# manycore-research/PlankAssembly

Measured on AMD Instinct MI355X. Metric: train samples/sec (fwd+bwd+all-reduce+Adam), d_model=512 seq=1024 [value: bf16 MFMA, f32 accumulate / master weights; train.f32 / train.x3: the same step in exact f32 / f32 with bf16x3 products = the parity paths], higher is better.
Workload: dtype bf16; 1 GPU; train_complete.yaml model d_model=512 H=8 dff=1024 6+6 post-norm layers, dropout 0.2, S=1024 (MAX_INPUT_LENGTH 1025), T=128, batch 16/GPU; global_batch=16, seq_len=1024, parallelism=dp1

## Files before the change

include/plank_hip.h:

```cpp
#ifndef PLANK_HIP_H
#define PLANK_HIP_H
#include <stdint.h>

#ifdef __cplusplus
extern "C" {
#endif

#define PA_F32 0
#define PA_BF16 1

#define PA_EINVAL (-1)
#define PA_EALIGN (-2)
#define PA_ESHAPE (-3)

int pa_version(void);

typedef struct {
    const void* A; const void* B; void* C;
    const float* bias;
    const void* R;
    const void* aux;
    void* ws;
    int32_t M, N, K;
    int32_t lda, ldb, ldc, ldr, ldaux;
    int64_t sA, sB, sC, sR, sAux;
    int32_t batch;
    int32_t a_kcontig, b_kcontig;
    int32_t in_dtype, out_dtype;
    float alpha;
    int32_t relu;
    float aux_scale;
    float drop_p; uint32_t drop_seed;
    int32_t splitk;
    int32_t splitk_defer;
    int64_t sBias;
    void* C_lp;
    int32_t ldc_lp; int32_t pad_lp_;
} pa_gemm_args;
int pa_gemm(const pa_gemm_args* a, void* stream);
int pa_set_reserved_cus(int32_t n);
int pa_get_reserved_cus(void);
int pa_gemm_effective_splitk(int32_t K, int32_t in_dtype, int32_t splitk);
int pa_split_ctx_create(void** out);
void pa_split_ctx_destroy(void* ctx);
int pa_split_ctx_enter(void* ctx);
void* pa_split_ctx_current(void);
int pa_gemm_split_config(int32_t on, void* ws, int64_t bytes);
int pa_gemm_split_active(void);
int64_t pa_gemm_split_reused(void);
int pa_gemm_split_stats(int64_t* out2, int32_t reset);
void* pa_gemm_split_reserve(const void* src, int32_t rows, int32_t cols, int32_t ld, int32_t* pat);
int64_t pa_gemm_split_made_hits(void);
int pa_gemm_split_cache_create(void* buf, int64_t bytes, void** out);
void pa_gemm_split_cache_destroy(void* cache);
// ... 31 lines not shown

typedef struct {
    const float* u; const float* gamma; const float* beta;
    void* y; int32_t ldy; float eps;
    const float* zf; int32_t ldzf; int32_t y_f32;
} pa_gemm_norm_ext;
int pa_ln_fold_weights(void* Wf, float* u, float* v, const float* W, const float* bias, const float* gamma, const float* beta,
                       int32_t N, int32_t K, void* stream);
int pa_gemm_norm_a(const pa_gemm_args* args, const pa_gemm_norm_ext* ext, void* stream);
int pa_gemm_plan(const pa_gemm_args* args, const pa_gemm_norm_ext* ext, pa_gemm_plan_info* out);
int pa_ln_fold_weights_f32(float* Wf, float* u, float* v, const float* W, const float* bias, const float* gamma, const float* beta,
                           int32_t N, int32_t K, void* stream);

#define PA_MAX_GROUP 8
int pa_gemm_group(const pa_gemm_args* args, int32_t n, void* stream);

#define PA_MAX_COLSUM 8
typedef struct {
    const void* X; float* out;
    int32_t M, N, ldx, pad_;
} pa_colsum_desc;
int pa_colsum_many(const pa_colsum_desc* descs, int32_t n_desc, int32_t dtype, void* stream);

#define PA_MAX_REDUCE 16
typedef struct {
    const float* ws; float* out;
    int32_t rows, cols, ld_out, splitk;
} pa_reduce_desc;
int pa_splitk_reduce_many(const pa_reduce_desc* descs, int32_t n_desc, void* stream);

// ... 220 lines not shown
```

plankassembly_amd/_lib.py:

```python
from __future__ import annotations

import ctypes as C
import os

import torch

HERE = os.path.dirname(os.path.abspath(__file__))
LIB_PATH = os.environ.get("PLANK_HIP_LIB") or os.path.join(HERE, "libplank_hip.so")

PA_F32, PA_BF16 = 0, 1
_ERR = {-1: "PA_EINVAL (bad argument)", -2: "PA_EALIGN (misaligned pointer / leading dimension)",
        -3: "PA_ESHAPE (unsupported shape)", -4: "PA_ESTATE (bad model/workspace state)"}


class PlankHipError(RuntimeError):
    pass


class GemmArgs(C.Structure):
    _fields_ = [("A", C.c_void_p), ("B", C.c_void_p), ("C", C.c_void_p), ("bias", C.c_void_p),
                ("R", C.c_void_p), ("aux", C.c_void_p), ("ws", C.c_void_p),
                ("M", C.c_int32), ("N", C.c_int32), ("K", C.c_int32),
                ("lda", C.c_int32), ("ldb", C.c_int32), ("ldc", C.c_int32), ("ldr", C.c_int32),
                ("ldaux", C.c_int32),
                ("sA", C.c_int64), ("sB", C.c_int64), ("sC", C.c_int64), ("sR", C.c_int64), ("sAux", C.c_int64),
                ("batch", C.c_int32), ("a_kcontig", C.c_int32), ("b_kcontig", C.c_int32),
                ("in_dtype", C.c_int32), ("out_dtype", C.c_int32), ("alpha", C.c_float), ("relu", C.c_int32),
                ("aux_scale", C.c_float), ("drop_p", C.c_float), ("drop_seed", C.c_uint32),
                ("splitk", C.c_int32), ("splitk_defer", C.c_int32), ("sBias", C.c_int64),
                ("C_lp", C.c_void_p), ("ldc_lp", C.c_int32), ("pad_lp_", C.c_int32)]


class GemmNormExt(C.Structure):
    _fields_ = [("u", C.c_void_p), ("gamma", C.c_void_p), ("beta", C.c_void_p), ("y", C.c_void_p),
                ("ldy", C.c_int32), ("eps", C.c_float),
                ("zf", C.c_void_p), ("ldzf", C.c_int32), ("y_f32", C.c_int32)]


class GemmPlanInfo(C.Structure):
    _fields_ = [("kind", C.c_int32), ("tile_h", C.c_int32), ("tile_w", C.c_int32), ("grid", C.c_int32),
                ("block", C.c_int32), ("splitk", C.c_int32), ("units", C.c_int32), ("pad_", C.c_int32)]


class GemmLnArgs(C.Structure):
    _fields_ = [("A", C.c_void_p), ("W", C.c_void_p), ("bias", C.c_void_p), ("R", C.c_void_p),
# ... 75 lines not shown
            "pa_gemm_split_config": (I, [I, P, I64]),
            "pa_gemm_split_stats": (I, [P, I]),
            "pa_gemm_split_reused": (I64, []),
            "pa_gemm_split_made_hits": (I64, []),
            "pa_gemm_split_cache_hits": (I64, []),
            "pa_gemm_split_reserve": (P, [P, I, I, I, P]),
            "pa_gemm_split_cache_create": (I, [P, I64, P]),
            "pa_gemm_split_cache_destroy": (None, [P]),
            "pa_gemm_split_cache_use": (I, [P]),
            "pa_gemm_split_cache_entries": (I, [P]),
            "pa_gemm_split_cache_refresh": (I, [P, P]),
            "pa_layernorm_fwd_img": (I, [P, P, P, P, P, P, I64, I, F, I, P, I, P]),
            "pa_layernorm_bwd_can_img": (I, [I, I]),
            "pa_layernorm_bwd_partial_img": (I, [P, P, P, P, P, P, P, I, P, I64, I, I, F, U, P, I, P]),
            "pa_gemm_group": (I, [P, I, P]),
            "pa_segment_tail": (I, [P, I, I, P, I, I, P, I, P]),
            "pa_gemm_record": (I, [I]),
            "pa_gemm_recorded": (I, [P, I]),
            "pa_gemm_recorded_kinds": (I, [P, I]),
            "pa_gemm_recorded_groups": (I, [P, I]),
            "pa_splitk_reduce_many": (I, [P, I, P]),
            "pa_colsum_many": (I, [P, I, I, P]),
            "pa_colsum_ws_floats": (I64, [I, I]),
            "pa_colsum": (I, [P, I, I, I, I, P, I, P, P]),
            "pa_embed_input_fwd": (I, [P, I, P, P, P, I, I64, I, P]),
            "pa_embed_input_bwd": (I, [P, I, P, P, P, P, I, I64, I, P]),
            "pa_embed_segment_bwd": (I, [P, I, P, P, P, P, I, I64, I, P]),
            "pa_pack_rows": (I, [P, I, I, P, P, P]),
            "pa_group_rows": (I, [P, I, P]),
            "pa_embed_output_fwd": (I, [P, I, P, P, P, P, I, I, I, I, I, P]),
# ... 51 lines not shown
            "pa_decode_sample_buffers": (I, [P, P]),
            "pa_decode_prefix_ws_bytes": (I64, [P, I, I]),
            "pa_decode_prefix_begin": (I, [P, P, P, P, P, I64, P]),
            "pa_decode_prefix_set": (I, [P, P, P, P, P]),
            "pa_decode_prefix_buffers": (I, [P, P, P]),
            "pa_dec_cross_mq": (I, [P, P, P, P, P, I, I, I, I, P]),
            "pa_dec_cross_mq32": (I, [P, P, P, P, P, I, I, I, I, P]),
            "pa_dec_cross_mq_ws": (I, [P, P, P, P, P, I, I, I, I, P, I64, P]),
            "pa_dec_cross_mq_ws_bytes": (I64, [I, I]),
            "pa_dec_cross_mq32_ws": (I, [P, P, P, P, P, I, I, I, I, P, I64, P]),
            "pa_dec_self_mq32": (I, [P, P, P, P, I, I, I, I, P]),
        }
        for name, (res, args) in sig.items():
            fn = getattr(_lib, name)
            fn.restype, fn.argtypes = res, args
    return _lib


class SampleParams(C.Structure):
    _fields_ = [("seed", C.c_uint32), ("n_per_drawing", C.c_int32), ("temperature", C.c_float), ("top_k", C.c_int32),
                ("top_p", C.c_float)]


def check(rc: int, what: str):
    if rc != 0:
        msg = _ERR.get(rc, f"hipError {rc}")
        raise PlankHipError(f"{what} failed: {msg}")


def ws_bytes(name: str, *args) -> int:
# ... 21 lines not shown
```

plankassembly_amd/csrc/gemm.hip:

```cpp
#include <stdlib.h>
#include <climits>
#include <atomic>
#include <new>
#include <mutex>
#include <vector>
#include <type_traits>
#include <utility>
#include "pa_device.h"
#include <mutex>
#include <vector>
#include "../../include/plank_hip.h"
#include "gemm_common.h"

namespace {

constexpr int BM = 128, BN = 128, NT = 256;
__device__ __attribute__((aligned(16))) const uint32_t pa_zero16[4] = {0u, 0u, 0u, 0u};
typedef short s16x4 __attribute__((ext_vector_type(4)));

#ifdef PA_GEMM_TRACE
__device__ unsigned long long pa_trace[8192];
__device__ int pa_trace_n;
#define TR_DECL __shared__ unsigned long long tr_lds[1024]; int tr_n = 0
#define TR(tag) do { if (blockIdx.x == 0 && threadIdx.x == 0 && tr_n < 1022) { tr_lds[tr_n++] = (unsigned long long)(tag); tr_lds[tr_n++] = __builtin_amdgcn_s_memtime(); } } while (0)
// ... 675 lines not shown
                TR(10);
                epilogue(c0.un, st);
                TR(11);
            }
            if (!has1) break;
            if (c1.u != c0.u) load_bias(c1.un);
            c0 = c1; c1 = c2;
            if (has2) advance(c2);
            st = (st + 1) % 3;
        }
        TR_FLUSH;
    }
}

constexpr int PA_MAX_GROUP_ = 8;
struct GemmGroup { GemmP p[PA_MAX_GROUP_]; int begin[PA_MAX_GROUP_ + 1]; int n; int xcd_chunk; };
__device__ __forceinline__ const GemmP& first_problem(const GemmP& p) { return p; }
__device__ __forceinline__ const GemmP& first_problem(const GemmGroup& g) { return g.p[0]; }
__device__ __forceinline__ int total_units_of(const GemmP& p) { return p.units; }
__device__ __forceinline__ int total_units_of(const GemmGroup& g) { return g.xcd_chunk > 0 ? 8 * g.xcd_chunk : g.begin[g.n]; }

#ifdef PA_GEMM_TRACE3
__device__ unsigned long long pa_gemm3_trace[512 * 8];
__device__ unsigned long long pa_gemm3_items[64];
__device__ int pa_gemm3_nitems;
#define PA_TR3(i) do { if (threadIdx.x == 0 && blockIdx.x < 512) pa_gemm3_trace[blockIdx.x * 8 + (i)] = __builtin_readcyclecounter(); } while (0)
#else
#define PA_TR3(i) do { } while (0)
#endif
template <bool A_KC, bool B_KC, typename PT>
__global__ __launch_bounds__(NT, 1) void gemm3_kernel(PT prm) {
// ... 8 lines not shown
    __shared__ __attribute__((aligned(256))) char smem[NSTG * STAGE + 4 * EPI];
    const int tid = threadIdx.x, lane = tid & 63;
    const int wave = __builtin_amdgcn_readfirstlane(tid >> 6);
    PA_TR3(0);
    const int wm = wave >> 1, wn = wave & 1;
    const int half = lane >> 5;
    constexpr int esz = 2;

    f32x16 acc[2][2];
#pragma unroll
    for (int i = 0; i < 2; ++i)
#pragma unroll
        for (int j = 0; j < 2; ++j)
#pragma unroll
            for (int r = 0; r < 16; ++r) acc[i][j][r] = 0.f;

    uint32_t offA[TL::NLD], offB[TL::NLD];
    bool okA[TL::NLD], okB[TL::NLD];
    const char* baseA = nullptr; const char* baseB = nullptr;
    auto setup = [&](const Unit& un) {
        baseA = reinterpret_cast<const char*>(pd.A) + (size_t)un.b * pd.sA * esz;
        baseB = reinterpret_cast<const char*>(pd.B) + (size_t)un.b * pd.sB * esz;
        const int m0 = un.tile_m * BM, n0 = un.tile_n * BN;
#pragma unroll
        for (int i = 0; i < TL::NLD; ++i) {
            const int pidx = tid + i * NT;
            if constexpr (A_KC) {
                const int row = pidx / TL::NCH, ch = ((pidx % TL::NCH) ^ (row / TL::RPB)) & (TL::NCH - 1);
                okA[i] = true;
                offA[i] = (uint32_t)min(m0 + row, pd.M - 1) * (uint32_t)(pd.lda * esz) + ch * 16;
// ... 97 lines not shown
#ifdef PA_GEMM_ABLATE
    const bool dbg_nomma = pc.dbg & 1, dbg_nord = pc.dbg & 2, dbg_nodma = pc.dbg & 4, dbg_nobar = pc.dbg & 8;
#define MMA1(ACC, X, Y) do { if (!dbg_nomma) PA_MFMA(ACC, X, Y); } while (0)
#define RD1(F, st, S, W) do { if (!dbg_nord) rd1(F, st, S, W); } while (0)
#define FRAG(F, st, S) do { if (!dbg_nord) frag(F, st, S); } while (0)
#define BAR() do { if (!dbg_nobar) __builtin_amdgcn_s_barrier(); } while (0)
#define DMA(x) do { if (!dbg_nodma) { x; } } while (0)
#else
#define MMA1(ACC, X, Y) PA_MFMA(ACC, X, Y)
#define RD1(F, st, S, W) rd1(F, st, S, W)
#define FRAG(F, st, S) frag(F, st, S)
#define BAR() __builtin_amdgcn_s_barrier()
#define DMA(x) do { x; } while (0)
#endif
    int sd = 0;
    auto step = [&](u32x4 (&fc)[4], u32x4 (&fn)[4], uint32_t stn, auto SN_, auto RD_, auto DQ_) {
        constexpr bool RD = decltype(RD_)::value;
        constexpr int DQ = decltype(DQ_)::value;
        wait_frag(fc);
        MMA1(acc[0][0], fc[2], fc[0]); if constexpr (RD) RD1(fn, stn, SN_, W0{});
        MMA1(acc[0][1], fc[2], fc[1]); if constexpr (RD) RD1(fn, stn, SN_, W1{});
        if constexpr (DQ >= 0) DMA(fetch_q(sd, std::integral_constant<int, (DQ >= 0 ? DQ : 0)>{}));
        MMA1(acc[1][0], fc[3], fc[0]); if constexpr (RD) RD1(fn, stn, SN_, W2{});
        MMA1(acc[1][1], fc[3], fc[1]); if constexpr (RD) RD1(fn, stn, SN_, W3{});
    };
    using NoQ = std::integral_constant<int, -1>;

    auto epilogue = [&](const Unit& un) {
        char* stage = smem + NSTG * STAGE + wave * EPI;
        const bool slab = pc.splitk > 1;
        const size_t cbase = slab ? (size_t)un.z * pc.M * pc.ldc : (size_t)un.b * pc.sC;
        const int mw = un.tile_m * BM + wm * 64, nw = un.tile_n * BN + wn * 64;
        const int chunk = lane & 15, rsub = lane >> 4;
        const int n = nw + chunk * 4;
        const bool out_f32 = slab || pc.out_dtype == PA_F32;
        const bool has_bias = !slab && pc.bias != nullptr, has_aux = !slab && pc.aux != nullptr;
        const bool has_res = !slab && pc.R != nullptr, has_drop = !slab && pc.drop_thr != 0;
        const bool fast = pc.vec_ok && (nw + 64 <= pc.N);
        const float alpha = slab ? 1.f : pc.alpha;
// ... 126 lines not shown
                        }
                        const size_t co = cbase + (size_t)m * pc.ldc + n + e;
                        if (out_f32) reinterpret_cast<float*>(pc.C)[co] = y;
                        else reinterpret_cast<bf16*>(pc.C)[co] = (bf16)y;
                    }
                }
            }
        }
#pragma unroll
        for (int i = 0; i < 2; ++i)
#pragma unroll
            for (int j = 0; j < 2; ++j)
#pragma unroll
                for (int r = 0; r < 16; ++r) acc[i][j][r] = 0.f;
    };

    const int ustride = gridDim.x;
    auto seek = [&](int u, Unit& un, GemmP& px, int& pi) -> int {
        while (u < total_units) {
            int local = u;
            if constexpr (GROUP) {
                int g = u;
                if (prm.xcd_chunk > 0) {
                    g = (u & 7) * prm.xcd_chunk + (u >> 3);
                    if (g >= prm.begin[prm.n]) { u += ustride; continue; }
                }
                bool moved = false;
                while (g >= prm.begin[pi + 1]) { ++pi; moved = true; }
                if (moved) px = prm.p[pi];
                local = g - prm.begin[pi];
// ... 11 lines not shown
        else cd_u = seek(u, un, pd, pd_i);
        if (cd_u < total_units) {
            setup(un);
            cd_t = un.t_begin; cd_end = un.t_end;
            k_dma = un.t_begin * TL::BK;
            stepA = A_KC ? (size_t)TL::BK * esz : (size_t)TL::BK * pd.lda * esz;
            stepB = B_KC ? (size_t)TL::BK * esz : (size_t)TL::BK * pd.ldb * esz;
            kA = baseA + (A_KC ? (size_t)k_dma * esz : (size_t)k_dma * pd.lda * esz);
            kB = baseB + (B_KC ? (size_t)k_dma * esz : (size_t)k_dma * pd.ldb * esz);
        }
    };
    Unit cun;
    auto cmp_enter = [&](int u) {
        cc_u = seek(u, cun, pc, pc_i);
        cc_t = cun.t_begin; cc_end = cun.t_end;
    };
    cmp_enter(blockIdx.x);
    if (cc_u >= total_units) return;
    dma_enter(cc_u, &cun);
    int pending = 0;
    auto issue = [&]() {
        DMA(fetch(sd));
        sd = (sd + 1) & (NSTG - 1);
        ++pending;
        if (++cd_t >= cd_end) dma_enter(cd_u + ustride);
    };
    auto wait_items = [&](int younger) {
        if (younger >= 2) asm volatile("s_waitcnt vmcnt(16)" ::: "memory");
        else if (younger == 1) asm volatile("s_waitcnt vmcnt(8)" ::: "memory");
        else asm volatile("s_waitcnt vmcnt(0)" ::: "memory");
    };
    PA_TR3(1);
#pragma unroll 1
    for (int k = 0; k < 3; ++k) if (cd_u < total_units) issue();
    wait_items(pending - 1);
    __builtin_amdgcn_s_barrier();
    PA_TR3(2);
    int sc = 0;
#ifdef PA_GEMM_TRACE3
    int tr_items = 0;
#endif
    u32x4 F0[4], F1[4];
    using S0 = std::integral_constant<int, 0>; using S1 = std::integral_constant<int, 1>;
    using S2 = std::integral_constant<int, 2>; using S3 = std::integral_constant<int, 3>;
    FRAG(F0, lds0, S0{});
    auto item = [&](auto HOT_) -> bool {
        constexpr bool HOT = decltype(HOT_)::value;
        using QA = std::integral_constant<int, HOT ? 0 : -1>; using QB = std::integral_constant<int, HOT ? 1 : -1>;
        using QC = std::integral_constant<int, HOT ? 2 : -1>; using QD = std::integral_constant<int, HOT ? 3 : -1>;
        const uint32_t st = lds0 + sc * STAGE;
#ifdef PA_GEMM_TRACE3
        if (threadIdx.x == 0 && blockIdx.x == 0 && tr_items < 63) pa_gemm3_items[tr_items++] = __builtin_readcyclecounter() | (HOT ? (1ull << 63) : 0ull);
#endif
        BAR();
        if constexpr (!HOT) { if (cd_u < total_units) issue(); }
        step(F0, F1, st, S1{}, std::true_type{}, QA{});
        step(F1, F0, st, S2{}, std::true_type{}, QB{});
        step(F0, F1, st, S3{}, std::true_type{}, QC{});
        const bool has_next = HOT || pending >= 2;
        if (has_next) {
            if constexpr (HOT) { DMA(fetch_q(sd, Q3{}); fetch_done()); sd = (sd + 1) & (NSTG - 1); ++cd_t; wait_items(2); }
            else wait_items(pending - 2);
            BAR();
        }
        step(F1, F0, lds0 + ((sc + 1) & (NSTG - 1)) * STAGE, S0{}, std::true_type{}, NoQ{});
        sc = (sc + 1) & (NSTG - 1);
        if constexpr (HOT) { ++cc_t; return true; }
        else {
            if (++cc_t >= cc_end) {
                PA_TR3(3);
#ifdef PA_GEMM_TRACE3
                if (threadIdx.x == 0 && blockIdx.x == 0) { pa_gemm3_items[tr_items] = __builtin_readcyclecounter(); pa_gemm3_nitems = tr_items; }
#endif
                epilogue(cun);
#ifdef PA_GEMM_TRACE3
                PA_TR3(5);
                asm volatile("s_waitcnt vmcnt(0)" ::: "memory");
#endif
                PA_TR3(4);
                if (has_next) cmp_enter(cc_u + ustride);
            }
            --pending;
            return has_next;
        }
    };
#pragma unroll 1
    while (true) {
        int hot = (pending == 3 && cd_u == cc_u) ? (cd_end - cd_t - 1) : 0;
#pragma unroll 1
        for (; hot > 0; --hot) item(std::true_type{});
        if (!item(std::false_type{})) break;
    }
#undef PA_RD128
#undef PA_RDTR
#undef MMA1
#undef RD1
#undef FRAG
#undef BAR
#undef DMA
#undef PA_MFMA
}

__global__ __launch_bounds__(NT, 2) void gemm3s_kernel(GemmP p) {
    using T = bf16;
    constexpr int TB = 64;
    constexpr int RB = 128, NCH = 8;
// ... 1056 lines not shown
inline GemmPlan plan_fail(int status) { GemmPlan pl = GemmPlan(); pl.status = status; return pl; }
inline void plan_kernel(GemmPlan& pl, int kind, GemmKernel kernel, const pa_gemm_args& a, int tile_h, int tile_w, int batch_times_splitk,
                        UnitOrder order, int max_blocks, int block) {
    pl.kind = kind; pl.kernel = kernel; pl.tile_h = tile_h; pl.tile_w = tile_w;
    pl.t = tiling_of(a.M, a.N, tile_h, tile_w, batch_times_splitk, order);
    pl.grid = pl.t.units < max_blocks ? pl.t.units : max_blocks;
    pl.block = block;
}

GemmPlan plan_gemm(const pa_gemm_args& a, const GemmSwitches& sw, int cus) {
    if (!a.A || !a.B || !a.C || a.M <= 0 || a.N <= 0 || a.K <= 0 || a.batch <= 0) return plan_fail(PA_EINVAL);
    if (a.in_dtype != PA_F32 && a.in_dtype != PA_BF16) return plan_fail(PA_EINVAL);
    if (a.out_dtype != PA_F32 && a.out_dtype != PA_BF16) return plan_fail(PA_EINVAL);
    if (a.drop_p < 0.f || a.drop_p >= 1.f) return plan_fail(PA_EINVAL);
    if (a.C_lp && (a.out_dtype != PA_F32 || a.ldc_lp < a.N || a.ldc_lp % 4 || (reinterpret_cast<uintptr_t>(a.C_lp) & 7))) return plan_fail(PA_EINVAL);
    GemmPlan pl = GemmPlan();
    const bool bf = a.in_dtype == PA_BF16, bk32 = bf && sw.bk == 32;
    pl.bk = bf ? (bk32 ? 32 : 64) : 16;
    const int nt = (a.K + pl.bk - 1) / pl.bk;
    const int splitk = eff_splitk(nt, a.splitk);
    if (splitk > 1 && !a.ws) return plan_fail(PA_EINVAL);
    pl.splitk = splitk;
    pl.tiles_per_slice = (nt + splitk - 1) / splitk;
    const int osz = (splitk > 1 || a.out_dtype == PA_F32) ? 4 : 2, isz = bf ? 2 : 4;
    pl.vec_ok = (splitk > 1 ? vec_ok(a.ws, a.N, (long long)a.M * a.N, osz) : vec_ok(a.C, a.ldc, a.sC, osz)) && vec_ok(a.R, a.ldr, a.sR, osz) &&
                vec_ok(a.aux, a.ldaux, a.sAux, isz) && vec_ok(a.bias, 4, a.sBias, 4);
    pl.aligned = bf ? is_aligned<bf16>(&a) : is_aligned<float>(&a);
    pl.glds = ((a.K % pl.bk) == 0 || (!a.a_kcontig && !a.b_kcontig && bf && !bk32)) && !sw.noglds;

    const Tiling base = tiling_of(a.M, a.N, BM, BN, a.batch * splitk, UNITS_XCD);
// ... 27 lines not shown
    }
    if (a.C_lp && !go_skinny) return plan_fail(PA_EINVAL);
    if (go_skinny) plan_kernel(pl, PA_GEMM_KIND_SKINNY, GK_SKINNY, a, SK_T, SK_T, 1, UNITS_PLAIN, INT_MAX, 256);
    else if (go_wide) plan_kernel(pl, PA_GEMM_KIND_WIDE, GK_WIDE, a, 128, 256, a.batch, UNITS_XCD_ALWAYS, cus, NT);
    else if (go_tall) plan_kernel(pl, PA_GEMM_KIND_WIDE, GK_TALL, a, 192, 128, a.batch, UNITS_XCD, cus, NT);
    else if (go_small) plan_kernel(pl, PA_GEMM_KIND_SMALL, GK_SMALL, a, 64, 64, a.batch, UNITS_PLAIN, 2 * cus, NT);
    else if (go_v3) plan_kernel(pl, PA_GEMM_KIND_RING, GK_RING, a, BM, BN, a.batch * splitk, UNITS_XCD, cus, NT);
    else {
        const int pair_cap = sw.grid > 0 ? (sw.grid / 256) * cus + sw.grid % 256 : INT_MAX;
        plan_kernel(pl, PA_GEMM_KIND_PAIR, GK_PAIR, a, BM, BN, a.batch * splitk, UNITS_XCD, pair_cap, NT);
    }
    return pl;
}

GemmPlan plan_norm_a(const pa_gemm_args& a, const pa_gemm_norm_ext& x, const GemmSwitches& sw, int cus) {
    if (!a.A || !a.B || !a.C || !a.bias || !x.u || a.M <= 0 || a.N <= 0 || a.K <= 0) return plan_fail(PA_EINVAL);
    if ((a.in_dtype != PA_BF16 && a.in_dtype != PA_F32) || (a.out_dtype != PA_BF16 && a.out_dtype != PA_F32) || !a.a_kcontig || !a.b_kcontig) return plan_fail(PA_EINVAL);
    auto al16 = [](const void* q) { return (reinterpret_cast<uintptr_t>(q) & 15) == 0; };
    GemmPlan pl = GemmPlan();
    pl.splitk = 1;
    const bool cbu_ok = vec_ok(a.C, a.ldc, 0, a.out_dtype == PA_F32 ? 4 : 2) && al16(a.bias) && al16(x.u);
    if (a.in_dtype == PA_F32) {
        if (a.batch != 1 || a.splitk > 1 || a.R || a.aux || a.drop_p != 0.f || a.N % 32) return plan_fail(PA_ESHAPE);
        if (!x.zf || a.K != 512 || a.M > sw.skinny_rows || a.out_dtype != PA_F32 || (x.y && (!x.y_f32 || a.N < a.K))) return plan_fail(PA_ESHAPE);
        if (x.y && (!x.gamma || !x.beta || x.ldy < a.K || x.ldy % 4 || !al16(x.y))) return plan_fail(PA_EINVAL);
        if (!is_aligned<float>(&a) || x.ldzf < a.K || x.ldzf % 4 || !al16(x.zf)) return plan_fail(PA_EALIGN);
        pl.vec_ok = cbu_ok && (!x.y || (al16(x.gamma) && al16(x.beta)));
        if (!pl.vec_ok) return plan_fail(PA_EALIGN);
        plan_kernel(pl, PA_GEMM_KIND_SKINNY, GK_SKINNY, a, SK_T, SK_T, 1, UNITS_PLAIN, INT_MAX, 256);
        return pl;
    }
// ... 577 lines not shown
        if (hb) { B3 = hb->dst; ++hits; }
        else { B3 = reinterpret_cast<bf16*>(g_split.ws + off); off += up(b_el * 2); job(a->B, B3, a->K, a->N, a->ldb, (inter ? 0 : 2) + 1 - pa); }
        b[i] = *a;
        b[i].in_dtype = PA_BF16; b[i].A = A3; b[i].B = B3; b[i].K = 3 * a->K; b[i].lda = a->M; b[i].ldb = a->N;
    }
    if (tb.n) PA_LAUNCH(split_kernel, dim3(tb.begin[tb.n]), dim3(256), 0, reinterpret_cast<hipStream_t>(stream), tb);
    g_split.on.store(0, std::memory_order_relaxed);
    const int rc = pa_gemm_group(b, n, stream);
    g_split.on.store(1, std::memory_order_relaxed);
    if (rc) return rc;
    g_cnt.taken.fetch_add(n);
    g_cnt.reused.fetch_add(hits);
    *taken = true;
    return 0;
}
extern "C" int pa_gemm_group(const pa_gemm_args* args, int32_t n, void* stream) {
    if (!args || n <= 0 || n > PA_MAX_GROUP) return PA_EINVAL;
    if (split_on() && args[0].in_dtype == PA_F32) {
        bool took = false;
        const int r3 = gemm_group_split3(args, n, stream, &took);
        if (r3) return r3;
        if (took) return 0;
        return PA_EINVAL;
    }
    static_assert(PA_MAX_GROUP == PA_MAX_GROUP_, "header / kernel table size");
    GemmGroup g; g.n = n; g.begin[0] = 0;
    int valid = 0;
    for (int i = 0; i < n; ++i) {
        const pa_gemm_args* a = &args[i];
        if (!a->A || !a->B || !a->C || a->M <= 0 || a->N <= 0 || a->K <= 0) return PA_EINVAL;
        if (a->in_dtype != PA_BF16 || a->out_dtype != PA_F32 || a->a_kcontig || a->b_kcontig || a->batch != 1) return PA_EINVAL;
        if (a->bias || a->R || a->aux || a->relu || a->drop_p > 0.f || a->alpha != 1.f) return PA_EINVAL;
        if (!is_aligned<bf16>(a)) return PA_EINVAL;
        const int nt = (a->K + 63) / 64, splitk = eff_splitk(nt, a->splitk);
        if (splitk > 1 && (!a->ws || !a->splitk_defer)) return PA_EINVAL;
        GemmP& p = g.p[i];
        p = GemmP{};
        fill_operands(p, *a);
        p.splitk = splitk; p.tiles_per_slice = (nt + splitk - 1) / splitk;
        set_tiling(p, BM, BN, splitk, UNITS_PLAIN);
        if (splitk > 1) { p.C = a->ws; p.ldc = a->N; }
        p.vec_ok = vec_ok(p.C, p.ldc, 0, 4);
        g.begin[i + 1] = g.begin[i] + p.units;
        valid += p.units;
        record_args(*a);
        record_kind(PA_GEMM_KIND_RING, g_rec_ngroups);
    }
    if (g_rec) { std::lock_guard<std::mutex> lk(g_rec_mu); if (g_rec) ++g_rec_ngroups; }
    const int cus = cus_for_gemm();
    int grid = valid < cus ? valid : cus;
    g.xcd_chunk = 0;
    if (gemm_switches().dw_xcd && valid >= 64) {
        g.xcd_chunk = (valid + 7) / 8;
        grid = (grid + 7) / 8 * 8;
        if (grid > 8 * g.xcd_chunk) grid = 8 * g.xcd_chunk;
    }
// ... 505 lines not shown
```

plankassembly_amd/csrc/runtime.hip:

```cpp
#include <stdlib.h>
#include <hip/hip_runtime.h>
#include <math.h>
#include <new>
#include <string.h>
#include <vector>
#include "../../include/plank_hip.h"

#include "model.h"

namespace {

#define RC(x) do { int rc_ = (x); if (rc_) return rc_; } while (0)

struct Ctx {
    pa_model* m; void* st;
    int dt() const { return m->cfg.dtype; }
    bool gelu() const { return m->cfg.activation == 2; }
    int ffn1(const void* A, const void* W, const float* bias, void* hidden, int rows, float drop_p, uint32_t seed) const {
        const int d = m->cfg.d_model, ff = m->cfg.d_ff;
        if (!gelu()) return linear(A, d, W, bias, hidden, ff, rows, ff, d, 1, drop_p, seed);
        RC(linear(A, d, W, bias, hidden, ff, rows, ff, d, 0));
        return pa_gelu_fwd(hidden, hidden, rows, ff, ff, dt(), drop_p, seed, st);
    }

// ... 21 lines not shown
    }
    int linear_dw(const void* dY, int lddy, const void* Xin, int ldx, float* dW, float* db, int M, int N, int K) const {
        pa_gemm_args g; memset(&g, 0, sizeof(g));
        g.A = dY; g.B = Xin; g.C = dW;
        g.M = N; g.N = K; g.K = M; g.lda = lddy; g.ldb = ldx; g.ldc = K;
        g.batch = 1; g.a_kcontig = 0; g.b_kcontig = 0;
        g.in_dtype = dt(); g.out_dtype = PA_F32;
        g.alpha = 1.f; g.aux_scale = 1.f;
        const int tiles = ((N + 127) / 128) * ((K + 127) / 128);
        const bool x3 = dt() == PA_F32 && pa_gemm_split_active();
        const int ktile = (dt() == PA_BF16 || x3) ? 64 : 16;
        const int nkt = ((x3 ? 3 * M : M) + ktile - 1) / ktile;
        static const bool plan = !(getenv("PA_DW_PLAN") && atoi(getenv("PA_DW_PLAN")) == 0);
        if (plan && m->defer_ok && tiles < 256 && m->ndwq < PA_MAX_GROUP) {
            g.splitk = 0; g.ws = nullptr;
            m->dwq[m->ndwq++] = g;
            return queue_bias(dY, lddy, db, M, N);
        }
        int sk = 1;
        if (tiles < 256) {
            static const int target_env = getenv("PA_DW_UNITS") ? atoi(getenv("PA_DW_UNITS")) : 0;
            const int target = target_env > 0 ? target_env : (m->defer_ok ? 64 : 256);
            sk = target / tiles > 0 ? target / tiles : 1;
            if (sk > 16) sk = 16;
            if (sk > nkt / 4) sk = nkt / 4 > 0 ? nkt / 4 : 1;
            while (sk > 1 && (size_t)sk * N * K > m->splitws_floats) --sk;
        }
        sk = pa_gemm_effective_splitk(M, dt(), sk);
        g.splitk = sk; g.ws = m->splitws;
        const size_t need = (size_t)sk * N * K;
        if (sk > 1 && m->ndefer < PA_MAX_REDUCE && m->slab_used + need <= m->splitws_floats && (K & 3) == 0) {
            g.ws = m->splitws + m->slab_used;
            g.splitk_defer = 1;
            pa_reduce_desc& rd = m->defer[m->ndefer++];
            rd.ws = m->splitws + m->slab_used; rd.out = dW; rd.rows = N; rd.cols = K; rd.ld_out = K; rd.splitk = sk;
            m->slab_used += (need + 3) / 4 * 4;
        }
        if (m->defer_ok && g.splitk_defer == (sk > 1 ? 1 : 0) && m->ndwq < PA_MAX_GROUP) {
            m->dwq[m->ndwq++] = g;
        } else {
            RC(pa_gemm(&g, st));
        }
        return queue_bias(dY, lddy, db, M, N);
    }
    int queue_bias(const void* dY, int lddy, float* db, int M, int N) const {
        if (db) {
            const int EB = dt() == PA_BF16 ? 8 : 4;
            const bool vec = (reinterpret_cast<uintptr_t>(dY) & 15) == 0 && lddy % EB == 0 && lddy >= (N + EB - 1) / EB * EB;
            if (m->defer_ok && vec && m->ncs < PA_MAX_COLSUM) {
                pa_colsum_desc& cd = m->cs[m->ncs++];
                cd.X = dY; cd.out = db; cd.M = M; cd.N = N; cd.ldx = lddy; cd.pad_ = 0;
            } else {
                RC(pa_colsum(dY, dt(), M, N, lddy, db, 1, m->partial, st));
            }
        }
        return 0;
    }
    int linear_ln(const void* A, int lda, const void* W, const float* bias, const void* R, void* z, void* y, const float* g,
                  const float* b, float* mean, float* rstd, int M, int K, float drop_p, uint32_t seed, float eps) const {
        static const int fuse_max = getenv("PLANK_TRAIN_FUSE_LN") ? atoi(getenv("PLANK_TRAIN_FUSE_LN")) : 0;
        const int d = m->cfg.d_model;
        if (dt() == PA_BF16 && d == 512 && M <= fuse_max && M <= pa_gemm_ln_max_rows() && K % 64 == 0) {
            pa_gemm_ln_args a; memset(&a, 0, sizeof(a));
            a.A = A; a.W = W; a.bias = bias; a.R = R; a.Z = z; a.Y = y; a.gamma = g; a.beta = b; a.mean = mean; a.rstd = rstd;
// ... 394 lines not shown
        pa_gemm_args& g = m->dwq[i];
        if (g.splitk > 0) continue;
        int s = pa_gemm_effective_splitk(g.K, g.in_dtype, sk[i]);
        const size_t need = (size_t)s * g.M * g.N;
        if (s > 1 && !(m->ndefer < PA_MAX_REDUCE && m->slab_used + need <= m->splitws_floats)) s = 1;
        g.splitk = s; g.ws = m->splitws; g.splitk_defer = 0;
        if (s > 1) {
            g.ws = m->splitws + m->slab_used;
            g.splitk_defer = 1;
            pa_reduce_desc& rd = m->defer[m->ndefer++];
            rd.ws = (const float*)g.ws; rd.out = (float*)g.C; rd.rows = g.M; rd.cols = g.N; rd.ld_out = g.ldc; rd.splitk = s;
            m->slab_used += (need + 3) / 4 * 4;
        }
    }
}
int flush_segment(pa_model* m, void* q) {
    if (m->ndwq > 0) {
        plan_group(m);
        int rc = m->ndwq > 1 ? pa_gemm_group(m->dwq, m->ndwq, q) : PA_EINVAL;
        if (rc == PA_EINVAL) { rc = 0; for (int i = 0; i < m->ndwq && !rc; ++i) rc = pa_gemm(&m->dwq[i], q); }
        m->ndwq = 0;
        RC(rc);
    }
    if (m->nlnq > 0 || m->ncs > 0 || m->ndefer > 0) {
        RC(pa_segment_tail(m->lnq, m->nlnq, m->cfg.d_model, m->cs, m->ncs, m->cfg.dtype, m->defer, m->ndefer, q));
        m->nlnq = 0; m->ncs = 0; m->ndefer = 0; m->slab_used = 0;
    }
    return 0;
}
int join_side(pa_model* m, int par, void* st) {
    if (m->ev_pending[par]) {
        HC(hipStreamWaitEvent((hipStream_t)st, (hipEvent_t)m->ev_done[par], 0));
        m->ev_pending[par] = false;
    }
// ... 233 lines not shown
```

plankassembly_amd/ops.py:

```python
from __future__ import annotations

import ctypes as C
import math

import torch

from . import _lib as L


def _f32(*shape, device):
    return torch.empty(*shape, dtype=torch.float32, device=device)


def gemm(a, b, *, a_kcontig=True, b_kcontig=True, bias=None, residual=None, aux=None, aux_scale=1.0,
         relu=False, alpha=1.0, drop_p=0.0, drop_seed=0, out_dtype=None, splitk=1, out=None, defer=False, out_lp=None):
    batched = a.dim() == 3
    A3 = a if batched else a[None]
    B3 = b if b.dim() == 3 else b[None]
    batch = A3.shape[0]
    M, K = (A3.shape[1], A3.shape[2]) if a_kcontig else (A3.shape[2], A3.shape[1])
    N = B3.shape[1] if b_kcontig else B3.shape[2]
    assert (B3.shape[2] if b_kcontig else B3.shape[1]) == K
    assert A3.stride(2) == 1 and B3.stride(2) == 1
    out_dtype = out_dtype or a.dtype
# ... 23 lines not shown
    if out_lp is not None:
        g.C_lp, g.ldc_lp = out_lp.data_ptr(), out_lp.stride(-2)
    splitk = int(L.lib().pa_gemm_effective_splitk(K, L.dt(a), splitk))
    g.splitk = splitk
    ws = None
    if splitk > 1:
        ws = _f32(splitk * batch * M * N, device=a.device)
        g.ws = ws.data_ptr()
        g.splitk_defer = int(defer)
    L.check(L.lib().pa_gemm(C.byref(g), L.stream()), "pa_gemm")
    if defer and splitk > 1:
        return out, ws, splitk
    return out


def dw_group(items):
    n = len(items)
    args = (L.GemmArgs * n)()
    outs, keep, red = [], [], []
    for i, (dy, x, sk) in enumerate(items):
        rows, M = dy.shape
        N = x.shape[1]
        sk = int(L.lib().pa_gemm_effective_splitk(rows, L.dt(dy), sk))
        out = torch.empty(M, N, dtype=torch.float32, device=dy.device)
        g = args[i]
        g.A, g.B, g.C = dy.data_ptr(), x.data_ptr(), out.data_ptr()
        g.M, g.N, g.K = M, N, rows
        g.lda, g.ldb, g.ldc = dy.stride(0), x.stride(0), out.stride(0)
        g.batch, g.a_kcontig, g.b_kcontig = 1, 0, 0
        g.in_dtype, g.out_dtype = L.dt(dy), L.dt(out)
        g.alpha, g.aux_scale, g.splitk = 1.0, 1.0, sk
        if sk > 1:
            ws = _f32(sk * M * N, device=dy.device)
            g.ws, g.splitk_defer = ws.data_ptr(), 1
            keep.append(ws)
            red.append((ws, out, sk))
        outs.append(out)
    L.check(L.lib().pa_gemm_group(C.cast(args, C.c_void_p), n, L.stream()), "pa_gemm_group")
    if red:
        splitk_reduce_many(red)
    return outs


class ColsumDesc(C.Structure):
    _fields_ = [("X", C.c_void_p), ("out", C.c_void_p), ("M", C.c_int32), ("N", C.c_int32), ("ldx", C.c_int32),
                ("pad_", C.c_int32)]


def colsum_many(items):
    n = len(items)
    descs = (ColsumDesc * n)()
    for i, (x, out) in enumerate(items):
        descs[i].X, descs[i].out = x.data_ptr(), out.data_ptr()
        descs[i].M, descs[i].N, descs[i].ldx = x.shape[0], x.shape[1], x.stride(0)
    L.check(L.lib().pa_colsum_many(C.cast(descs, C.c_void_p), n, L.dt(items[0][0]), L.stream()), "pa_colsum_many")


class ReduceDesc(C.Structure):
    _fields_ = [("ws", C.c_void_p), ("out", C.c_void_p), ("rows", C.c_int32), ("cols", C.c_int32),
                ("ld_out", C.c_int32), ("splitk", C.c_int32)]


def splitk_reduce_many(items):
    n = len(items)
    descs = (ReduceDesc * n)()
    for i, (ws, out, sk) in enumerate(items):
        descs[i].ws, descs[i].out = ws.data_ptr(), out.data_ptr()
        descs[i].rows, descs[i].cols, descs[i].ld_out, descs[i].splitk = out.shape[0], out.shape[1], out.stride(0), sk
    L.check(L.lib().pa_splitk_reduce_many(C.cast(descs, C.c_void_p), n, L.stream()), "pa_splitk_reduce_many")


def colsum(x, out=None, accumulate=False):
    M, N = x.shape
    if out is None:
        out = torch.zeros(N, dtype=torch.float32, device=x.device)
    part = _f32(int(L.lib().pa_colsum_ws_floats(M, N)), device=x.device)
    L.check(L.lib().pa_colsum(L.ptr(x), L.dt(x), M, N, x.stride(0), L.ptr(out), int(accumulate), L.ptr(part),
                              L.stream()), "pa_colsum")
    return out


def _ptr_array(tensors):
# ... 295 lines not shown
```

Baseline: 3329 samples/s.

## Fuse bias-gradient column sums into grouped dW GEMM via ones-vector MFMA

Computes the bias gradient inside the grouped weight-gradient GEMM by issuing extra MFMAs against a vector of bf16 ones while the dY fragments are already in registers. Only the tile_n==0 waves accumulate it. Split-K partials go to a workspace reduced alongside the weight partials, and the fallback path returns to a separate colsum kernel. This is meant to remove the separate colsum pass that rereads dY, at the cost of extra MFMA work, more registers in the hot loop for tile_n==0 blocks, and more launch-planning logic.

New measurement: 1060 samples/s. 68.1% lower.

```diff
diff --git a/include/plank_hip.h b/include/plank_hip.h
--- a/include/plank_hip.h
+++ b/include/plank_hip.h
@@ -36,8 +36,10 @@
     int64_t sBias;
     void* C_lp;
     int32_t ldc_lp; int32_t pad_lp_;
+    float* db; float* db_ws;
 } pa_gemm_args;
 int pa_gemm(const pa_gemm_args* a, void* stream);
+int32_t pa_gemm_args_size(void);
 int pa_set_reserved_cus(int32_t n);
 int pa_get_reserved_cus(void);
 int pa_gemm_effective_splitk(int32_t K, int32_t in_dtype, int32_t splitk);
@@ -99,6 +101,7 @@
 
 #define PA_MAX_GROUP 8
 int pa_gemm_group(const pa_gemm_args* args, int32_t n, void* stream);
+int pa_gemm_group_check(const pa_gemm_args* args, int32_t n);
 
 #define PA_MAX_COLSUM 8
 typedef struct {
diff --git a/plankassembly_amd/_lib.py b/plankassembly_amd/_lib.py
--- a/plankassembly_amd/_lib.py
+++ b/plankassembly_amd/_lib.py
@@ -28,7 +28,8 @@
                 ("in_dtype", C.c_int32), ("out_dtype", C.c_int32), ("alpha", C.c_float), ("relu", C.c_int32),
                 ("aux_scale", C.c_float), ("drop_p", C.c_float), ("drop_seed", C.c_uint32),
                 ("splitk", C.c_int32), ("splitk_defer", C.c_int32), ("sBias", C.c_int64),
-                ("C_lp", C.c_void_p), ("ldc_lp", C.c_int32), ("pad_lp_", C.c_int32)]
+                ("C_lp", C.c_void_p), ("ldc_lp", C.c_int32), ("pad_lp_", C.c_int32),
+                ("db", C.c_void_p), ("db_ws", C.c_void_p)]
 
 
 class GemmNormExt(C.Structure):
@@ -134,6 +135,8 @@
             "pa_layernorm_bwd_can_img": (I, [I, I]),
             "pa_layernorm_bwd_partial_img": (I, [P, P, P, P, P, P, P, I, P, I64, I, I, F, U, P, I, P]),
             "pa_gemm_group": (I, [P, I, P]),
+            "pa_gemm_group_check": (I, [P, I]),
+            "pa_gemm_args_size": (I, []),
             "pa_segment_tail": (I, [P, I, I, P, I, I, P, I, P]),
             "pa_gemm_record": (I, [I]),
             "pa_gemm_recorded": (I, [P, I]),
@@ -215,6 +218,9 @@
         for name, (res, args) in sig.items():
             fn = getattr(_lib, name)
             fn.restype, fn.argtypes = res, args
+        if _lib.pa_gemm_args_size() != C.sizeof(GemmArgs):
+            raise PlankHipError(f"{LIB_PATH}: pa_gemm_args is {_lib.pa_gemm_args_size()} bytes, the GemmArgs mirror "
+                                f"{C.sizeof(GemmArgs)}: the library and this package are different versions")
     return _lib
 
 
diff --git a/plankassembly_amd/csrc/gemm.hip b/plankassembly_amd/csrc/gemm.hip
--- a/plankassembly_amd/csrc/gemm.hip
+++ b/plankassembly_amd/csrc/gemm.hip
@@ -713,7 +713,7 @@
 }
 
 constexpr int PA_MAX_GROUP_ = 8;
-struct GemmGroup { GemmP p[PA_MAX_GROUP_]; int begin[PA_MAX_GROUP_ + 1]; int n; int xcd_chunk; };
+struct GemmGroup { GemmP p[PA_MAX_GROUP_]; int begin[PA_MAX_GROUP_ + 1]; int n; int xcd_chunk; float* db[PA_MAX_GROUP_]; float* db_ws[PA_MAX_GROUP_]; };
 __device__ __forceinline__ const GemmP& first_problem(const GemmP& p) { return p; }
 __device__ __forceinline__ const GemmP& first_problem(const GemmGroup& g) { return g.p[0]; }
 __device__ __forceinline__ int total_units_of(const GemmP& p) { return p.units; }
@@ -752,6 +752,18 @@
         for (int j = 0; j < 2; ++j)
 #pragma unroll
             for (int r = 0; r < 16; ++r) acc[i][j][r] = 0.f;
+    f32x16 accb[2];
+    u32x4 ones;
+    bool bias_on = false;
+    float* db_c = nullptr; float* dbws_c = nullptr;
+    if constexpr (GROUP) {
+#pragma unroll
+        for (int i = 0; i < 2; ++i)
+#pragma unroll
+            for (int r = 0; r < 16; ++r) accb[i][r] = 0.f;
+#pragma unroll
+        for (int e = 0; e < 4; ++e) ones[e] = 0x3f803f80u;
+    }
 
     uint32_t offA[TL::NLD], offB[TL::NLD];
     bool okA[TL::NLD], okB[TL::NLD];
@@ -879,8 +891,9 @@
 #define DMA(x) do { x; } while (0)
 #endif
     int sd = 0;
-    auto step = [&](u32x4 (&fc)[4], u32x4 (&fn)[4], uint32_t stn, auto SN_, auto RD_, auto DQ_) {
+    auto step = [&](u32x4 (&fc)[4], u32x4 (&fn)[4], uint32_t stn, auto SN_, auto RD_, auto DQ_, auto BIAS_) {
         constexpr bool RD = decltype(RD_)::value;
+        constexpr bool BIAS = decltype(BIAS_)::value;
         constexpr int DQ = decltype(DQ_)::value;
         wait_frag(fc);
         MMA1(acc[0][0], fc[2], fc[0]); if constexpr (RD) RD1(fn, stn, SN_, W0{});
@@ -888,6 +901,7 @@
         if constexpr (DQ >= 0) DMA(fetch_q(sd, std::integral_constant<int, (DQ >= 0 ? DQ : 0)>{}));
         MMA1(acc[1][0], fc[3], fc[0]); if constexpr (RD) RD1(fn, stn, SN_, W2{});
         MMA1(acc[1][1], fc[3], fc[1]); if constexpr (RD) RD1(fn, stn, SN_, W3{});
+        if constexpr (BIAS) { MMA1(accb[0], ones, fc[0]); MMA1(accb[1], ones, fc[1]); }
     };
     using NoQ = std::integral_constant<int, -1>;
 
@@ -1044,6 +1058,16 @@
 #pragma unroll
                 for (int r = 0; r < 16; ++r) acc[i][j][r] = 0.f;
     };
+    auto bias_epilogue = [&](const Unit& un) {
+        float* dst = pc.splitk > 1 ? dbws_c + (size_t)un.z * pc.M : db_c;
+        const int m = un.tile_m * BM + wm * 64 + (lane & 31);
+#pragma unroll
+        for (int i = 0; i < 2; ++i) {
+            if (lane < 32 && m + i * 32 < pc.M) dst[m + i * 32] = accb[i][0];
+#pragma unroll
+            for (int r = 0; r < 16; ++r) accb[i][r] = 0.f;
+        }
+    };
 
     const int ustride = gridDim.x;
     auto seek = [&](int u, Unit& un, GemmP& px, int& pi) -> int {
@@ -1085,6 +1109,10 @@
     auto cmp_enter = [&](int u) {
         cc_u = seek(u, cun, pc, pc_i);
         cc_t = cun.t_begin; cc_end = cun.t_end;
+        if constexpr (GROUP) {
+            if (cc_u < total_units) { db_c = prm.db[pc_i]; dbws_c = prm.db_ws[pc_i]; }
+            bias_on = wn == 0 && db_c != nullptr && cc_u < total_units && cun.tile_n == 0;
+        }
     };
     cmp_enter(blockIdx.x);
     if (cc_u >= total_units) return;
@@ -1115,7 +1143,7 @@
     using S0 = std::integral_constant<int, 0>; using S1 = std::integral_constant<int, 1>;
     using S2 = std::integral_constant<int, 2>; using S3 = std::integral_constant<int, 3>;
     FRAG(F0, lds0, S0{});
-    auto item = [&](auto HOT_) -> bool {
+    auto item = [&](auto HOT_, auto BIAS_) -> bool {
         constexpr bool HOT = decltype(HOT_)::value;
         using QA = std::integral_constant<int, HOT ? 0 : -1>; using QB = std::integral_constant<int, HOT ? 1 : -1>;
         using QC = std::integral_constant<int, HOT ? 2 : -1>; using QD = std::integral_constant<int, HOT ? 3 : -1>;
@@ -1125,16 +1153,16 @@
 #endif
         BAR();
         if constexpr (!HOT) { if (cd_u < total_units) issue(); }
-        step(F0, F1, st, S1{}, std::true_type{}, QA{});
-        step(F1, F0, st, S2{}, std::true_type{}, QB{});
-        step(F0, F1, st, S3{}, std::true_type{}, QC{});
+        step(F0, F1, st, S1{}, std::true_type{}, QA{}, BIAS_);
+        step(F1, F0, st, S2{}, std::true_type{}, QB{}, BIAS_);
+        step(F0, F1, st, S3{}, std::true_type{}, QC{}, BIAS_);
         const bool has_next = HOT || pending >= 2;
         if (has_next) {
             if constexpr (HOT) { DMA(fetch_q(sd, Q3{}); fetch_done()); sd = (sd + 1) & (NSTG - 1); ++cd_t; wait_items(2); }
             else wait_items(pending - 2);
             BAR();
         }
-        step(F1, F0, lds0 + ((sc + 1) & (NSTG - 1)) * STAGE, S0{}, std::true_type{}, NoQ{});
+        step(F1, F0, lds0 + ((sc + 1) & (NSTG - 1)) * STAGE, S0{}, std::true_type{}, NoQ{}, BIAS_);
         sc = (sc + 1) & (NSTG - 1);
         if constexpr (HOT) { ++cc_t; return true; }
         else {
@@ -1144,6 +1172,7 @@
                 if (threadIdx.x == 0 && blockIdx.x == 0) { pa_gemm3_items[tr_items] = __builtin_readcyclecounter(); pa_gemm3_nitems = tr_items; }
 #endif
                 epilogue(cun);
+                if constexpr (decltype(BIAS_)::value) bias_epilogue(cun);
 #ifdef PA_GEMM_TRACE3
                 PA_TR3(5);
                 asm volatile("s_waitcnt vmcnt(0)" ::: "memory");
@@ -1158,9 +1187,17 @@
 #pragma unroll 1
     while (true) {
         int hot = (pending == 3 && cd_u == cc_u) ? (cd_end - cd_t - 1) : 0;
+        if constexpr (GROUP) {
+            if (bias_on) {
 #pragma unroll 1
-        for (; hot > 0; --hot) item(std::true_type{});
-        if (!item(std::false_type{})) break;
+                for (; hot > 0; --hot) item(std::true_type{}, std::true_type{});
+                if (!item(std::false_type{}, std::true_type{})) break;
+                continue;
+            }
+        }
+#pragma unroll 1
+        for (; hot > 0; --hot) item(std::true_type{}, std::false_type{});
+        if (!item(std::false_type{}, std::false_type{})) break;
     }
 #undef PA_RD128
 #undef PA_RDTR
@@ -2247,6 +2284,7 @@
     if (a.out_dtype != PA_F32 && a.out_dtype != PA_BF16) return plan_fail(PA_EINVAL);
     if (a.drop_p < 0.f || a.drop_p >= 1.f) return plan_fail(PA_EINVAL);
     if (a.C_lp && (a.out_dtype != PA_F32 || a.ldc_lp < a.N || a.ldc_lp % 4 || (reinterpret_cast<uintptr_t>(a.C_lp) & 7))) return plan_fail(PA_EINVAL);
+    if (a.db || a.db_ws) return plan_fail(PA_EINVAL);
     GemmPlan pl = GemmPlan();
     const bool bf = a.in_dtype == PA_BF16, bk32 = bf && sw.bk == 32;
     pl.bk = bf ? (bk32 ? 32 : 64) : 16;
@@ -2304,7 +2342,7 @@
 }
 
 GemmPlan plan_norm_a(const pa_gemm_args& a, const pa_gemm_norm_ext& x, const GemmSwitches& sw, int cus) {
-    if (!a.A || !a.B || !a.C || !a.bias || !x.u || a.M <= 0 || a.N <= 0 || a.K <= 0) return plan_fail(PA_EINVAL);
+    if (!a.A || !a.B || !a.C || !a.bias || !x.u || a.M <= 0 || a.N <= 0 || a.K <= 0 || a.db || a.db_ws) return plan_fail(PA_EINVAL);
     if ((a.in_dtype != PA_BF16 && a.in_dtype != PA_F32) || (a.out_dtype != PA_BF16 && a.out_dtype != PA_F32) || !a.a_kcontig || !a.b_kcontig) return plan_fail(PA_EINVAL);
     auto al16 = [](const void* q) { return (reinterpret_cast<uintptr_t>(q) & 15) == 0; };
     GemmPlan pl = GemmPlan();
@@ -2912,9 +2950,26 @@
     *taken = true;
     return 0;
 }
+static int group_member_status(const pa_gemm_args* a) {
+    if (!a->A || !a->B || !a->C || a->M <= 0 || a->N <= 0 || a->K <= 0) return PA_EINVAL;
+    if (a->in_dtype != PA_BF16 || a->out_dtype != PA_F32 || a->a_kcontig || a->b_kcontig || a->batch != 1) return PA_EINVAL;
+    if (a->bias || a->R || a->aux || a->relu || a->drop_p > 0.f || a->alpha != 1.f) return PA_EINVAL;
+    if (!is_aligned<bf16>(a)) return PA_EINVAL;
+    const int splitk = eff_splitk((a->K + 63) / 64, a->splitk);
+    if (splitk > 1 && (!a->ws || !a->splitk_defer)) return PA_EINVAL;
+    if (a->db ? (splitk > 1 && (!a->db_ws || (reinterpret_cast<uintptr_t>(a->db_ws) & 15))) : a->db_ws != nullptr) return PA_EINVAL;
+    return 0;
+}
+extern "C" int pa_gemm_group_check(const pa_gemm_args* args, int32_t n) {
+    if (!args || n <= 0 || n > PA_MAX_GROUP) return PA_EINVAL;
+    for (int i = 0; i < n; ++i) { const int rc = group_member_status(&args[i]); if (rc) return rc; }
+    return 0;
+}
+extern "C" int32_t pa_gemm_args_size(void) { return (int32_t)sizeof(pa_gemm_args); }
 extern "C" int pa_gemm_group(const pa_gemm_args* args, int32_t n, void* stream) {
     if (!args || n <= 0 || n > PA_MAX_GROUP) return PA_EINVAL;
     if (split_on() && args[0].in_dtype == PA_F32) {
+        for (int i = 0; i < n; ++i) if (args[i].db || args[i].db_ws) return PA_EINVAL;
         bool took = false;
         const int r3 = gemm_group_split3(args, n, stream, &took);
         if (r3) return r3;
@@ -2926,18 +2981,15 @@
     int valid = 0;
     for (int i = 0; i < n; ++i) {
         const pa_gemm_args* a = &args[i];
-        if (!a->A || !a->B || !a->C || a->M <= 0 || a->N <= 0 || a->K <= 0) return PA_EINVAL;
-        if (a->in_dtype != PA_BF16 || a->out_dtype != PA_F32 || a->a_kcontig || a->b_kcontig || a->batch != 1) return PA_EINVAL;
-        if (a->bias || a->R || a->aux || a->relu || a->drop_p > 0.f || a->alpha != 1.f) return PA_EINVAL;
-        if (!is_aligned<bf16>(a)) return PA_EINVAL;
+        if (const int rc = group_member_status(a)) return rc;
         const int nt = (a->K + 63) / 64, splitk = eff_splitk(nt, a->splitk);
-        if (splitk > 1 && (!a->ws || !a->splitk_defer)) return PA_EINVAL;
         GemmP& p = g.p[i];
         p = GemmP{};
         fill_operands(p, *a);
         p.splitk = splitk; p.tiles_per_slice = (nt + splitk - 1) / splitk;
         set_tiling(p, BM, BN, splitk, UNITS_PLAIN);
         if (splitk > 1) { p.C = a->ws; p.ldc = a->N; }
+        g.db[i] = a->db; g.db_ws[i] = a->db_ws;
         p.vec_ok = vec_ok(p.C, p.ldc, 0, 4);
         g.begin[i + 1] = g.begin[i] + p.units;
         valid += p.units;
diff --git a/plankassembly_amd/csrc/runtime.hip b/plankassembly_amd/csrc/runtime.hip
--- a/plankassembly_amd/csrc/runtime.hip
+++ b/plankassembly_amd/csrc/runtime.hip
@@ -59,6 +59,7 @@
         static const bool plan = !(getenv("PA_DW_PLAN") && atoi(getenv("PA_DW_PLAN")) == 0);
         if (plan && m->defer_ok && tiles < 256 && m->ndwq < PA_MAX_GROUP) {
             g.splitk = 0; g.ws = nullptr;
+            if (bias_from_group(db)) { g.db = db; db = nullptr; }
             m->dwq[m->ndwq++] = g;
             return queue_bias(dY, lddy, db, M, N);
         }
@@ -82,17 +83,22 @@
             m->slab_used += (need + 3) / 4 * 4;
         }
         if (m->defer_ok && g.splitk_defer == (sk > 1 ? 1 : 0) && m->ndwq < PA_MAX_GROUP) {
+            if (bias_from_group(db)) { g.db = db; db = nullptr; }
             m->dwq[m->ndwq++] = g;
         } else {
             RC(pa_gemm(&g, st));
         }
         return queue_bias(dY, lddy, db, M, N);
     }
-    int queue_bias(const void* dY, int lddy, float* db, int M, int N) const {
+    bool bias_from_group(const float* db) const {
+        static const bool on = !(getenv("PA_DW_BIAS") && atoi(getenv("PA_DW_BIAS")) == 0);
+        return on && db && dt() == PA_BF16 && (reinterpret_cast<uintptr_t>(db) & 15) == 0;
+    }
+    int queue_bias(const void* dY, int lddy, float* db, int M, int N, bool at_flush = false) const {
         if (db) {
             const int EB = dt() == PA_BF16 ? 8 : 4;
             const bool vec = (reinterpret_cast<uintptr_t>(dY) & 15) == 0 && lddy % EB == 0 && lddy >= (N + EB - 1) / EB * EB;
-            if (m->defer_ok && vec && m->ncs < PA_MAX_COLSUM) {
+            if ((m->defer_ok || at_flush) && vec && m->ncs < PA_MAX_COLSUM) {
                 pa_colsum_desc& cd = m->cs[m->ncs++];
                 cd.X = dY; cd.out = db; cd.M = M; cd.N = N; cd.ldx = lddy; cd.pad_ = 0;
             } else {
@@ -517,10 +523,42 @@
         }
     }
 }
+bool dw_group_on() {
+    static const bool on = !(getenv("PA_DW_GROUP") && atoi(getenv("PA_DW_GROUP")) == 0);
+    return on;
+}
+int plan_bias(pa_model* m, void* q) {
+    const int ndefer0 = m->ndefer; const size_t slab0 = m->slab_used;
+    Ctx k{m, q};
+    auto to_colsum = [&](pa_gemm_args& g) {
+        float* db = g.db;
+        g.db = nullptr; g.db_ws = nullptr;
+        return k.queue_bias(g.A, g.lda, db, g.K, g.M, true);
+    };
+    for (int i = 0; i < m->ndwq; ++i) {
+        pa_gemm_args& g = m->dwq[i];
+        if (!g.db || g.splitk <= 1) continue;
+        const size_t need = (size_t)g.splitk * g.M;
+        if ((g.M & 3) == 0 && m->ndefer < PA_MAX_REDUCE && m->slab_used + need <= m->splitws_floats) {
+            g.db_ws = m->splitws + m->slab_used;
+            pa_reduce_desc& rd = m->defer[m->ndefer++];
+            rd.ws = g.db_ws; rd.out = g.db; rd.rows = 1; rd.cols = g.M; rd.ld_out = g.M; rd.splitk = g.splitk;
+            m->slab_used += (need + 3) / 4 * 4;
+        } else {
+            RC(to_colsum(g));
+        }
+    }
+    if (dw_group_on() && m->ndwq > 1 && pa_gemm_group_check(m->dwq, m->ndwq) == 0) return 0;
+    m->ndefer = ndefer0; m->slab_used = slab0;
+    for (int i = 0; i < m->ndwq; ++i)
+        if (m->dwq[i].db) RC(to_colsum(m->dwq[i]));
+    return 0;
+}
 int flush_segment(pa_model* m, void* q) {
     if (m->ndwq > 0) {
         plan_group(m);
-        int rc = m->ndwq > 1 ? pa_gemm_group(m->dwq, m->ndwq, q) : PA_EINVAL;
+        RC(plan_bias(m, q));
+        int rc = dw_group_on() && m->ndwq > 1 ? pa_gemm_group(m->dwq, m->ndwq, q) : PA_EINVAL;
         if (rc == PA_EINVAL) { rc = 0; for (int i = 0; i < m->ndwq && !rc; ++i) rc = pa_gemm(&m->dwq[i], q); }
         m->ndwq = 0;
         RC(rc);
diff --git a/plankassembly_amd/ops.py b/plankassembly_amd/ops.py
--- a/plankassembly_amd/ops.py
+++ b/plankassembly_amd/ops.py
@@ -61,7 +61,7 @@
     return out
 
 
-def dw_group(items):
+def dw_group(items, bias=None, bias_ws=None):
     n = len(items)
     args = (L.GemmArgs * n)()
     outs, keep, red = [], [], []
@@ -83,6 +83,25 @@
             keep.append(ws)
             red.append((ws, out, sk))
         outs.append(out)
+    want = [i for i in range(n) if bias is not None and bias[i] is not None]
+    if want:
+        for i in want:
+            g, M = args[i], bias[i].numel()
+            g.db = bias[i].data_ptr()
+            if g.splitk > 1:
+                pw = bias_ws[i] if bias_ws is not None and bias_ws[i] is not None else _f32(g.splitk * M, device=bias[i].device)
+                g.db_ws = pw.data_ptr()
+                keep.append(pw)
+        if n == 1 or L.lib().pa_gemm_group_check(C.cast(args, C.c_void_p), n) != 0:
+            for i in range(n):
+                args[i].db = args[i].db_ws = None
+                L.check(L.lib().pa_gemm(C.byref(args[i]), L.stream()), "pa_gemm")
+            if red:
+                splitk_reduce_many(red)
+            for i in want:
+                colsum(items[i][0], out=bias[i], accumulate=False)
+            return outs
+        red += [(C.c_void_p(args[i].db_ws), bias[i].view(1, -1), args[i].splitk) for i in want if args[i].splitk > 1]
     L.check(L.lib().pa_gemm_group(C.cast(args, C.c_void_p), n, L.stream()), "pa_gemm_group")
     if red:
         splitk_reduce_many(red)
@@ -112,7 +131,7 @@
     n = len(items)
     descs = (ReduceDesc * n)()
     for i, (ws, out, sk) in enumerate(items):
-        descs[i].ws, descs[i].out = ws.data_ptr(), out.data_ptr()
+        descs[i].ws, descs[i].out = (ws.value if isinstance(ws, C.c_void_p) else ws.data_ptr()), out.data_ptr()
         descs[i].rows, descs[i].cols, descs[i].ld_out, descs[i].splitk = out.shape[0], out.shape[1], out.stride(0), sk
     L.check(L.lib().pa_splitk_reduce_many(C.cast(descs, C.c_void_p), n, L.stream()), "pa_splitk_reduce_many")
 
```
